# richox/orz

Measured on AMD Instinct MI355X. Metric: orz -l1 encode throughput (enwik8-shaped text, 100 MB, one 16 MiB block in flight), higher is better.
Workload: dtype u8

## Files before the change

### orz_amd/csrc/backend_hip.h

```cpp
#pragma once
#include <hip/hip_runtime.h>

#include <cxxabi.h>

#include <chrono>
#include <condition_variable>
#include <algorithm>
#include <atomic>
#include <cstring>
#include <map>
#include <mutex>
#include <rocprim/rocprim.hpp>
#include <stdexcept>
#include <string>
#include <type_traits>
#include <vector>

#include "orz_kernels.h"
#include "orz_parse.h"
#include "orz_symrank.h"

namespace orz {

#define ORZ_HIP_CHECK(expr)                                                                              \
// ... 32 lines not shown
        const uint32_t lo = (uint32_t)__builtin_amdgcn_readlane((int)(uint32_t)v, (int)src);
        const uint32_t hi = (uint32_t)__builtin_amdgcn_readlane((int)(uint32_t)(v >> 32), (int)src);
        return (uint64_t)lo | ((uint64_t)hi << 32);
    }
    __device__ __forceinline__ unsigned long long clock() const { return __builtin_amdgcn_s_memtime(); }
    __device__ __forceinline__ unsigned long long wallclock() const { return __builtin_amdgcn_s_memrealtime(); }
};
template <class K>
__global__ __launch_bounds__(64) void orz_wave_kernel(K k) {
    extern __shared__ __attribute__((aligned(16))) uint8_t orz_dyn_lds[];
    DevWave w{orz_dyn_lds};
    k(w);
}

template <class K>
__global__ __launch_bounds__(1024) void orz_group_kernel(K k, bool use_lds) {
    extern __shared__ __attribute__((aligned(16))) uint8_t orz_dyn_lds[];
    for (uint32_t ph = 0; ph < K::kPhases; ph++) {
        if (ph) {
            __threadfence_block();
            __syncthreads();
        }
        k.phase(ph, threadIdx.x, blockDim.x, orz_dyn_lds, use_lds);
    }
}

__global__ __launch_bounds__(256) void orz_rank_kernel(RankArgs a, uint32_t nchunks, uint32_t nvblk) {
    __shared__ uint32_t rows[(kRankChunk + 1) * 256];
    auto sync = [] __device__() { __syncthreads(); };
    if (blockIdx.x < nchunks) rank_chunk(a, blockIdx.x, threadIdx.x, rows, sync);
    else if (blockIdx.x < nchunks + nvblk)
        rebuild_summaries(a.vbits, a.v1, a.v2, a.nvwords, blockIdx.x - nchunks, threadIdx.x, (uint64_t*)rows, sync);
    else
        rebuild_summaries(a.kbits, a.k1, a.k2, a.nkwords, blockIdx.x - nchunks - nvblk, threadIdx.x, (uint64_t*)rows, sync);
}


struct FastEval;

class ParseTokens {
   public:
    static ParseTokens& of(int device) {
        static ParseTokens t[64];
        return t[device & 63];
    }
    void acquire() {
// ... 281 lines not shown
        static std::atomic<int> done[64];
        std::atomic<int>* d = device_ >= 0 && device_ < 64 ? &done[device_] : nullptr;
        if (d) {
            const int v = d->load(std::memory_order_acquire);
            if (v) return (hipError_t)(v - 1);
        }
        int cur = -1;
        ORZ_HIP_CHECK(hipGetDevice(&cur));
        if (cur != device_) ORZ_HIP_CHECK(hipSetDevice(device_));
        const hipError_t e = hipFuncSetAttribute(reinterpret_cast<const void*>(Kernel), hipFuncAttributeMaxDynamicSharedMemorySize, bytes);
        if (cur != device_) ORZ_HIP_CHECK(hipSetDevice(cur));
        if (d) d->store(1 + (int)e, std::memory_order_release);
        return e;
    }
    template <class K>
    void launch_waves(size_t nblocks, const K& k, size_t lds_bytes) {
        if (!nblocks) return;
        Bracket br(*this, profile_ ? KernelNames::of<K>() : 0);
        if (lds_bytes > 64 * 1024) {
            const hipError_t big = big_lds<&orz_wave_kernel<K>>(160 * 1024 - 256);
            if (big != hipSuccess) throw std::runtime_error(std::string("hipFuncSetAttribute(MaxDynamicSharedMemorySize): ") + hipGetErrorString(big));
        }
        hipLaunchKernelGGL(orz_wave_kernel<K>, dim3((unsigned)nblocks), dim3(64), lds_bytes, stream_, k);
        ORZ_HIP_CHECK(hipGetLastError());
    }
    template <class K>
    void launch_group(const K& k) {
        Bracket br(*this, profile_ ? KernelNames::of<K>() : 0);
        size_t lds = k.lds_bytes();
        const bool big_ok = big_lds<&orz_group_kernel<K>>((int)K::kLdsMax) == hipSuccess;
        if (lds > 64 * 1024 && !big_ok) lds = 0;
        hipLaunchKernelGGL(orz_group_kernel<K>, dim3(1), dim3(1024), lds, stream_, k, lds != 0);
        ORZ_HIP_CHECK(hipGetLastError());
    }
    void huffbuild(const HuffBuild& f) {
        if (f.nchunks) launch_waves((size_t)f.nchunks * 3, HuffWave{f}, HuffWave::lds_bytes());
    }
    void rank(const RankArgs& a, uint32_t nchunks) {
        const uint32_t nvblk = (a.nvwords + 4095) / 4096, nkblk = (a.nkwords + 4095) / 4096;
        hipLaunchKernelGGL(orz_rank_kernel, dim3(nchunks + nvblk + nkblk), dim3(256), 0, stream_, a, nchunks, nvblk);
        ORZ_HIP_CHECK(hipGetLastError());
    }
    void sort_pairs_u32(const uint32_t* kin, uint32_t* kout, const uint32_t* vin, uint32_t* vout, size_t n, int bits) {
        if (n == 0) return;
        Bracket br(*this, profile_ ? KernelNames::lib("(radix sort, pairs)") : 0);
        size_t sz = tmp_bytes_;
// ... 229 lines not shown
```

### orz_amd/csrc/orz_fast.h

```cpp
#pragma once
#include "orz_kernels.h"
#include "orz_parse.h"

namespace orz {

#if !defined(__HIPCC__)
inline unsigned long long g_far_stats[4] = {0, 0, 0, 0};
#endif

constexpr uint32_t kSub = 4096;
constexpr uint32_t kSeg64 = 64;
constexpr uint32_t kNSub = kNewMax / kSub + 2;
constexpr uint32_t kEntries = 240;

constexpr uint32_t kFastK = 32;
constexpr uint32_t kHistSub = (kPre + 1) / kSub;
constexpr uint32_t kRingMargin = 4;
constexpr uint32_t kFastTile = 262144;
constexpr uint32_t kFastRounds = 4;
constexpr uint32_t kSettledTile = 393216;
constexpr uint32_t kSettledTileDeep = 262144;
constexpr uint32_t kSettledRounds = 3;

struct FastArgs {
    const uint8_t* win;
    uint32_t len, n;
    uint32_t K, depth, lazy1, lazy2, tile;
    uint32_t dmax;
    uint32_t nent, nk;
    const uint32_t *idx, *epos, *kidx, *kpos, *krun;
    const uint8_t* rows;
    const uint8_t* rlen;
    const uint64_t* rdist;
    const uint64_t* wmask;
    const uint16_t* kmeta;
    const uint16_t* kw;
    const uint8_t* wsnap;
    const uint32_t* ORD;
    const uint64_t* stext;
    const uint32_t* runstart;
    const uint32_t* hpre;
    uint32_t far;
    uint32_t near;
    uint32_t near1;
    uint32_t extra;
    uint64_t* cl;
    uint32_t *ccnt, *cnew;
    uint32_t rounds;
    uint32_t* farv;
    uint64_t *vbits, *kbits;
    uint64_t* v1;
    uint64_t* k1;
    uint64_t* tbits;
    uint32_t* ev;
    uint8_t *ty, *nl, *pt;
    uint64_t* sbits;
    uint8_t *mfb, *efb;
    uint8_t* dirty;
// ... 166 lines not shown
            }
        }
        if (p < kPre) return;
        const uint32_t d = j - rs;
        rlen[p - kPre] = (uint8_t)(d < 255 ? d : 255);
    }
};
struct FastKw {
    const uint8_t* win;
    const uint32_t* kpos;
    uint32_t nk;
    uint16_t* kw;
    ORZ_HD void operator()(size_t s) const {
        if (s >= nk) return;
        const uint32_t u = kpos[s];
        kw[s] = (uint16_t)(win[u] | (win[u + 1] << 8));
    }
};
struct FastWordMasks {
    const uint32_t *kpos, *kkeys, *krun;
    const uint16_t* kw;
    const uint8_t* wsnap;
    uint32_t nk;
    uint64_t* wmask;
    uint16_t* kmeta;
    static size_t lds_bytes() { return 128 * 2; }
    template <class W>
    ORZ_D void operator()(W& w) const {
        uint16_t* kwL = (uint16_t*)w.lds();
        const uint32_t lane = w.lane();
        const int64_t base = (int64_t)w.block() * 64 - 64;
        for (uint32_t e = lane; e < 128; e += 64) {
            const int64_t s = base + e;
            kwL[e] = s >= 0 && s < (int64_t)nk ? kw[s] : 0;
        }
        w.sync();
        const uint32_t s = w.block() * 64 + lane;
        if (s >= nk) return;
        const uint32_t u = kpos[s];
        if (u < kPre) return;
        const uint32_t key = kkeys[s], rk = fast_min(64u, s - krun[key]);
        const uint32_t me = 64 + lane, wv = kwL[me];
        uint64_t m = 0;
        for (uint32_t t = 0; t < rk; t++) m |= (uint64_t)(kwL[me - 1 - t] == wv) << (63 - t);
        const uint32_t excl = rk && kpos[s - 1] == u - 1;
        const uint32_t snap = ((uint32_t)wsnap[key * 2] | ((uint32_t)wsnap[key * 2 + 1] << 8)) == wv;
        wmask[u - kPre] = m;
        kmeta[u - kPre] = (uint16_t)(rk | (excl << 7) | (snap << 8));
    }
};
struct HistCountWave {
    const uint8_t* win;
    const uint8_t* S;
    uint32_t* hcm;
    static size_t lds_bytes() { return 256 * 4; }
    template <class W>
    ORZ_D void operator()(W& w) const {
        uint32_t* cnt = (uint32_t*)w.lds();
        const uint32_t u = w.block(), lane = w.lane();
        for (uint32_t c = lane; c < 256; c += 64) cnt[c] = 0;
        w.sync();
        const uint32_t x0 = u * kSub + lane * 64;
        for (uint32_t k = 0; k < 64; k++) {
            const uint32_t x = x0 + k - 1;
            if (x0 + k == 0 || x < 1 || x >= kPre) continue;
            if (S[x]) atom_add32(&cnt[hash1(win, x - 1)], 1);
        }
        w.sync();
        for (uint32_t c = lane; c < 256; c += 64) hcm[(size_t)u * 256 + c] = cnt[c];
    }
};
// ... 40 lines not shown
        uint32_t v = gsum[(size_t)g * 256 + c];
        for (uint32_t r = g * 64; r < rows && r < g * 64 + 64; r++) {
            out[(size_t)r * 256 + c] = v;
            v += in[(size_t)r * 256 + c];
        }
        if (g * 64 + 64 >= rows) out[(size_t)rows * 256 + c] = v;
    }
};
constexpr uint32_t kRecText = 12;
ORZ_D uint32_t rec_pos(uint64_t hi) { return (uint32_t)(hi >> 32); }
ORZ_D uint32_t rec_lcp(uint64_t lo_a, uint64_t hi_a, uint64_t lo_b, uint64_t hi_b) {
    const uint64_t x0 = lo_a ^ lo_b;
    if (x0) return (uint32_t)ctz64(x0) >> 3;
    const uint32_t x1 = (uint32_t)(hi_a ^ hi_b);
    return x1 ? 8 + ((uint32_t)ctz64((uint64_t)x1) >> 3) : kRecText;
}
struct FastRowsWave {
    const uint8_t* win;
    const uint32_t* epos;
    const uint64_t* stext;
    const uint8_t* rlen;
    uint32_t nent, K;
    uint8_t* rows;
    uint64_t* rdist;
    static constexpr uint32_t kOutStride = 72;
    static size_t lds_bytes(uint32_t K) { return (size_t)(64 + K) * 16 + 64 * kOutStride; }
    template <class W>
    ORZ_D void operator()(W& w) const {
        uint64_t* t0 = (uint64_t*)w.lds();
        uint64_t* t1 = t0 + (64 + K);
        uint8_t* outL = (uint8_t*)(t1 + (64 + K));
        const uint32_t lane = w.lane();
        const int64_t base = (int64_t)w.block() * 64 - K;
        for (uint32_t e = lane; e < 64 + K; e += 64) {
            const int64_t s = base + e;
            uint64_t a = 0, b = 0;
            if (s >= 0 && s < (int64_t)nent) { a = stext[2 * s]; b = stext[2 * s + 1]; }
            t0[e] = a; t1[e] = b;
        }
        w.sync();
        const uint32_t me = K + lane;
        const uint32_t p = rec_pos(t1[me]);
        const bool mine = (int64_t)w.block() * 64 + lane < (int64_t)nent && p >= kPre;
        const uint32_t r = mine ? fast_min(K, rlen[p - kPre]) : 0;
        const uint64_t a0 = t0[me], a1 = t1[me];
        const uint64_t a2 = mine ? ldu64(win + p + kRecText) : 0;
        if (mine) {
            uint64_t codes = 0;
            for (uint32_t m = 0; m < 8; m++) {
                const uint32_t k = r ? fast_min(dist_sample(m), r - 1) : 0;
                const uint32_t code = r ? dist_code_up(p - rec_pos(t1[me - 1 - k])) : 255u;
                codes |= (uint64_t)code << (8 * m);
            }
            rdist[p - kPre] = codes;
        }
        const uint32_t cols = K < 64 ? K : 64;
        const uint32_t parts = cols / 16;
        for (uint32_t c0 = 0; c0 < K; c0 += cols) {
            for (uint32_t k0 = 0; k0 < cols; k0 += 8) {
                uint32_t ll[8], lq[8];
                uint64_t yy[8];
#pragma unroll
                for (uint32_t kk = 0; kk < 8; kk++) {
                    const uint32_t k = c0 + k0 + kk;
                    ll[kk] = 0; lq[kk] = 0;
                    if (k < r) {
                        const uint32_t e = me - 1 - k;
                        const uint64_t hi = t1[e];
                        ll[kk] = rec_lcp(t0[e], hi, a0, a1);
                        lq[kk] = rec_pos(hi);
                    }
                }
#pragma unroll
                for (uint32_t kk = 0; kk < 8; kk++) yy[kk] = ll[kk] == kRecText ? ldu64(win + lq[kk] + kRecText) : 0;
                uint64_t pack = 0;
#pragma unroll
                for (uint32_t kk = 0; kk < 8; kk++) {
// ... 251 lines not shown
                    else if (rnd == a.rounds) {
                        g_scan_hist[1][sb]++;
                        if (a.farv[i] != fv) { g_scan_hist[2][sb]++; g_scan_hist[3][popc64(wbits) < 63 ? popc64(wbits) : 63]++; }
                    }
                }
#endif
        }
        return fv;
    }
    ORZ_D uint32_t position_of(size_t tid) const {
        const uint32_t span = hi - lo, T = a.tile;
        if ((a.dbg & 2048) || span <= T) return lo + (uint32_t)tid;
        const uint32_t nch = (span + T - 1) / T, s_last = span - (nch - 1) * T;
        if (tid < s_last) return lo + (nch - 1) * T + (uint32_t)tid;
        const uint32_t u = (uint32_t)tid - s_last, k = u / T, off = u - k * T;
        const uint32_t c = k == 0 ? nch - 2 : k - 1;
        return lo + c * T + off;
    }
    ORZ_HD void operator()(size_t tid) const {
        const uint32_t p = position_of(tid);
        if (p >= hi) return;
        const uint8_t* win = a.win;
        const uint32_t i = p - kPre;
        const uint32_t rl = a.rlen[i];
        const bool first = p >= r1lo;
        const bool longrun = rl > kFastK;
        const uint32_t t = i / a.tile, rnd = step > t ? step - t : 0;
        bool scan = longrun && (rnd <= 1 || rnd == a.rounds);
        if (a.dbg & (12 | 128 | 256)) {
            if ((a.dbg & 8) || ((a.dbg & 4) && rnd > 1)) scan = false;
            if ((a.dbg & 128) && rnd <= 1) scan = false;
            if (a.dbg & 256) scan = longrun && (rnd == 2 || rnd == a.rounds);
        }
        if ((a.dbg & 16) && scan && rnd > 1) {
            const uint64_t sw = bits_at(a.sbits, (int64_t)i - 2);
            const bool rel = ((sw >> 2) & 1) || (((sw >> 1) & 1) && i >= 1 && a.ty[i - 1] == kTyMatch) || ((sw & 1) && i >= 2 && a.ty[i - 2] == kTyMatch);
            if (!rel) scan = false;
        }
        const bool dirty = a.dirty[i] != 0 || (a.dbg & 1);
        const uint32_t c = hash1(win, p - 1);
        const uint32_t* hz = a.hz + ((size_t)(i / kSub) * 256 + c) * 4;
        const uint32_t h4 = hz[0], h4was = hz[2];
        const bool need = p >= r2lo || dirty || scan;
#if !defined(__HIPCC__) && !defined(ORZ_EMU_THREADS)
        g_eval_stats[0]++;
        if (first) g_eval_stats[2]++; else if (dirty) g_eval_stats[3]++; else if (scan) g_eval_stats[4]++;
#endif
        if (!need && h4was == h4) return;
        const uint64_t codes = a.rdist[i];
        const DistBracket d4 = dist_valid(codes, p > h4 ? p - h4 : 0);
        bool moved = false;
        if (!first && h4was != h4) {
            const DistBracket o4 = dist_valid(codes, p > h4was ? p - h4was : 0);
            moved = o4.sure != d4.sure || o4.limit != d4.limit || d4.sure < fast_min(fast_min(kFastK, rl), d4.limit);
        }
        if (!need && !moved) return;
#if !defined(__HIPCC__) && !defined(ORZ_EMU_THREADS)
        g_eval_stats[1]++;
#endif
        const uint32_t j = a.idx[p], kj = a.kidx[p], r = fast_min(kFastK, rl);
        const uint32_t km = a.kmeta[i], rk = km & 0x7f;
        const uint64_t wm = a.wmask[i];
        const uint32_t h5 = hz[1];
        uint32_t rw[kFastK / 4];
        {
            const uint32_t* src = reinterpret_cast<const uint32_t*>(a.rows + (size_t)i * kFastK);
#pragma unroll
            for (uint32_t q = 0; q < kFastK / 16; q++) {
                if (r > q * 16) {
#pragma unroll
                    for (uint32_t d = 0; d < 4; d++) rw[q * 4 + d] = src[q * 4 + d];
                } else {
#pragma unroll
                    for (uint32_t d = 0; d < 4; d++) rw[q * 4 + d] = 0;
                }
            }
        }
        uint64_t mask = r ? bits_at(a.vbits, (int64_t)j - 64) : 0;
        uint64_t kmask = rk ? bits_at(a.kbits, (int64_t)kj - 64) : 0;
        if (r < 64) mask = r ? mask & (~0ull << (64 - r)) : 0;
        const uint64_t wbits = mask;
        const DistBracket d5 = dist_valid(codes, p > h5 ? p - h5 : 0);
        uint32_t v4 = count_from(d4, r, j, h4);
        if (a.dbg & 2) v4 = 64;
        const uint32_t span = fast_min(r, v4);
// ... 201 lines not shown
    uint32_t c0, nc;
    ORZ_HD void operator()(size_t tid) const {
        const uint32_t c = c0 + (uint32_t)(tid / kEntries), e = (uint32_t)(tid % kEntries);
        if (c >= c0 + nc) return;
        const uint32_t end = chunk_end(c, a.len);
        uint32_t x = kPre + c * kSub + e;
        while (x < end) {
            const uint32_t s = (x - kPre) / kSeg64;
            x = seg_end(s, a.len) + a.x0[x - kPre];
        }
        a.x1[(size_t)c * kEntries + e] = (uint8_t)(x >= end ? x - end : 0);
    }
};
ORZ_D uint32_t pad68(uint32_t x) { return (x >> 6) * 68 + (x & 63); }
ORZ_D void st8_pad68(uint8_t* tab, uint32_t x, uint64_t v) {
    uint32_t* d = reinterpret_cast<uint32_t*>(tab + pad68(x));
    d[0] = (uint32_t)v; d[1] = (uint32_t)(v >> 32);
}
struct PathUpWave {
    FastArgs a;
    uint32_t c0;
    uint32_t decide = 0, nup = 0;
    FastRetireDone done{};
    static size_t lds_bytes() { return 2 * 64 * 68 + 64; }
    template <class W>
    ORZ_D void operator()(W& w) const {
        if (decide && w.block() >= nup) {
            const uint32_t t = (w.block() - nup) * 64 + w.lane();
            done((size_t)t);
            return;
        }
        uint8_t* nlL = w.lds();
        uint8_t* x0L = nlL + 64 * 68 + 32;
        const uint32_t c = c0 + w.block() / 4, part = w.block() & 3, lane = w.lane();
        const uint32_t cs = kPre + c * kSub, clen = chunk_end(c, a.len) - cs;
        uint64_t w5[8][5];
        if (decide) {
#pragma unroll
            for (uint32_t k = 0; k < 8; k++) {
                const uint32_t x = (k * 64 + lane) * 8;
                const uint64_t* ew = reinterpret_cast<const uint64_t*>(a.ev + (cs - kPre) + (x < clen ? x : 0));
#pragma unroll
                for (uint32_t q = 0; q < 5; q++) w5[k][q] = ew[q];
            }
        }
#pragma unroll
        for (uint32_t k = 0; k < 8; k++) {
            const uint32_t x = (k * 64 + lane) * 8;
            if (!decide) {
                st8_pad68(nlL, x, x < clen ? *reinterpret_cast<const uint64_t*>(a.nl + (cs - kPre) + x) : 0);
                continue;
            }
            uint64_t nlw = 0, tyw = 0;
            if (x < clen) {
                const uint32_t i0 = (cs - kPre) + x;
                uint32_t e[10];
#pragma unroll
                for (uint32_t q = 0; q < 10; q++) {
                    const uint32_t v = (uint32_t)(w5[k][q >> 1] >> (32 * (q & 1)));
                    e[q] = cs + x + q < a.len ? v : 0;
                }
#pragma unroll
                for (uint32_t q = 0; q < 8; q++) {
                    const uint32_t p = cs + x + q;
                    const uint32_t d = p < a.len ? fast_decide(p, a.len, e[q], e[q + 1], e[q + 2]) : 0;
                    tyw |= (uint64_t)(d & 0xff) << (8 * q);
                    nlw |= (uint64_t)((d >> 8) & 0xff) << (8 * q);
                }
                if ((x >> 10) == part) {
                    if (x + 8 <= clen) {
                        *reinterpret_cast<uint64_t*>(a.ty + i0) = tyw;
                        *reinterpret_cast<uint64_t*>(a.nl + i0) = nlw;
                    } else {
                        for (uint32_t q = 0; x + q < clen; q++) { a.ty[i0 + q] = (uint8_t)(tyw >> (8 * q)); a.nl[i0 + q] = (uint8_t)(nlw >> (8 * q)); }
                    }
                }
            }
            st8_pad68(nlL, x, nlw);
        }
        w.sync();
        {
            const uint32_t s0 = lane * 64;
            if (s0 < clen) {
                const uint32_t s1 = fast_min(s0 + 64, clen), sl = s1 - s0;
                uint32_t adv[16];
                const uint32_t* row = reinterpret_cast<const uint32_t*>(nlL + lane * 68);
#pragma unroll
                for (uint32_t q = 0; q < 16; q++) adv[q] = row[q];
                uint8_t* xrow = x0L + lane * 68;
#pragma unroll
                for (uint32_t k = 0; k < 64; k++) {
                    const uint32_t p = 63 - k;
                    if (p < sl) {
                        const uint32_t d = (adv[p >> 2] >> (8 * (p & 3))) & 0xff, x = p + (d ? d : 1);
                        xrow[p] = x >= sl ? (uint8_t)(x - sl) : xrow[x];
                    }
                }
            }
        }
        w.sync();
        for (uint32_t k = part * 2; k < part * 2 + 2; k++) {
            const uint32_t x = (k * 64 + lane) * 8;
            if (x >= clen) continue;
            const uint32_t* src = reinterpret_cast<const uint32_t*>(x0L + pad68(x));
            *reinterpret_cast<uint64_t*>(a.x0 + (cs - kPre) + x) = (uint64_t)src[0] | ((uint64_t)src[1] << 32);
        }
        w.sync();
        if (lane < 60) {
            const uint32_t e = part * 60 + lane;
            uint32_t x = e;
            while (x < clen) {
                const uint32_t s1 = fast_min(((x >> 6) + 1) * 64, clen);
                x = s1 + x0L[pad68(x)];
            }
            a.x1[(size_t)c * kEntries + e] = (uint8_t)(x - clen);
        }
    }
};
struct PathMarkWave {
    FastArgs a;
    uint32_t c0;
    static constexpr uint32_t kTab = 64 * 68 + 32;
    static size_t lds_bytes() { return 3 * kTab + (65 * 68 + 12) + 256 * 4; }
    template <class W>
    ORZ_D void operator()(W& w) const {
        uint8_t* nlL = w.lds();
        uint8_t* x0L = nlL + kTab;
        uint8_t* tyL = x0L + kTab;
        uint8_t* wL = tyL + kTab;
        uint32_t* cnt = (uint32_t*)(wL + 65 * 68 + 12);
        const uint32_t c = c0 + w.block(), lane = w.lane();
        const uint32_t cs = kPre + c * kSub, clen = chunk_end(c, a.len) - cs;
        for (uint32_t k = lane; k < 256; k += 64) cnt[k] = 0;
        {
            uint64_t v[8], u[8], t[8], b[8];
#pragma unroll
            for (uint32_t k = 0; k < 8; k++) {
                const uint32_t x = (k * 64 + lane) * 8;
// ... 966 lines not shown
```

### orz_amd/csrc/orz_stream.h

```cpp
#pragma once
#include <algorithm>
#include <atomic>
#include <cstdio>
#include <cstdlib>
#include <cstring>
#include <stdexcept>
#include <string>
#include <vector>

#include "orz_fast.h"
#include "orz_kernels.h"
#include "orz_parse.h"
#include "orz_verify.h"

namespace orz {

struct ItemTrace {
    std::vector<uint32_t> block, pos, src;
    std::vector<uint16_t> sym, ctx, rank, rob;
    std::vector<uint8_t> unl, enc, al, mlen;
    void clear() { block.clear(); pos.clear(); src.clear(); sym.clear(); ctx.clear(); rank.clear(); rob.clear(); unl.clear(); enc.clear(); al.clear(); mlen.clear(); }
};

struct FastTableCapture {
// ... 316 lines not shown
        n_ = m;
    }
    void push_back(uint8_t b) {
        if (n_ == cap_) reserve(cap_ ? cap_ * 2 : 4096);
        p_[n_++] = b;
    }
    size_t size() const { return n_; }
    bool empty() const { return n_ == 0; }
    uint8_t* data() { return p_; }
    const uint8_t* data() const { return p_; }
    void clear() { n_ = 0; }
    uint8_t* release() {
        if (!p_) reserve(1);
        uint8_t* q = p_;
        p_ = nullptr;
        n_ = cap_ = 0;
        return q;
    }

   private:
    uint8_t* p_ = nullptr;
    size_t n_ = 0, cap_ = 0;
};

template <class BE>
class StreamEncoder {
   public:
    static constexpr size_t kChunkCapWords = (size_t)kChunkItems * 40 / 32 + 8192;
    static constexpr uint32_t kMaxChunks = 17;
    static constexpr uint32_t kNumKeys = 256 * kHash;
    static constexpr uint32_t kDirtyWords = kNumKeys / 64 + 1;
    static constexpr int kFirstPasses = 12;
    static constexpr uint32_t kRepairGrid = 16384;

    StreamEncoder(BE& be, Cfg cfg, uint32_t seg_size = 62, uint32_t win_segs = 3072, bool fast = false,
                  uint32_t fast_tile = kFastTile, uint32_t fast_rounds = kFastRounds)
        : be_(be), cfg_(cfg), seg_(seg_size), wsegs_(win_segs), fast_(fast), ftile_(fast_tile), frounds_(fast_rounds) {
        if (fast_) {
            if (ftile_ < kSub || ftile_ % kSub || ftile_ > kNewMax) throw std::runtime_error("fast tile must be a multiple of 4096 in [4096, 16777216]");
            if (frounds_ < 1 || frounds_ > 64) throw std::runtime_error("fast rounds must be in [1, 64]");
            fK_ = kFastK;
            sched_auto_ = ftile_ == kFastTile && frounds_ == kFastRounds;
            if (cfg.depth > 20) sched_tile_ = kSettledTileDeep;
            if (const char* sc = getenv("ORZ_FAST_SCHED")) {
                unsigned t = 0, r = 0;
                if (sscanf(sc, "%ux%u", &t, &r) == 2 && t >= kSub && t % kSub == 0 && t <= kNewMax && r >= 1 && r <= 64) { sched_tile_ = t; sched_rounds_ = r; }
// ... 55 lines not shown
            kbits_ = take<uint64_t>(kNewMax / 64 + 2);
            k1_ = take<uint64_t>(kNewMax / 4096 + 2);
            k2_ = take<uint64_t>(kNewMax / 262144 + 2);
            if (!fast_) {
                srec_ = take<SlotRec>(kWLen);
                exitst_ = take<uint64_t>((size_t)nseg_max_ + 2);
                hist_ = take<uint8_t>((size_t)ring_ * 256);
                base_ = take<uint32_t>((size_t)ring_ * 256);
                ctl_ = take<ParseCtl>(1);
                partial_ = take<uint32_t>((size_t)2 * (wsegs_ / kRankChunk + 1) * 256);
            } else {
                const size_t nn = (size_t)kNewMax + 512;
                frows_ = take<uint8_t>((size_t)kNewMax * fK_ + 64, false);
                frlen_ = take<uint8_t>(nn);
                fstext_ = take<uint64_t>((size_t)kWLen * 2, false);
                fkw_ = take<uint16_t>(nn);
                fev_ = take<uint32_t>(nn, false);
                fty_ = take<uint8_t>(nn);
                fnl_ = take<uint8_t>(nn);
                fpt_ = take<uint8_t>(nn);
                fmf_ = take<uint8_t>(nn);
                fef_ = take<uint8_t>(nn);
                fdirty_ = take<uint8_t>(nn);
                frdist_ = take<uint64_t>(nn, false);
                fwmask_ = take<uint64_t>(nn, false);
                fkmeta_ = take<uint16_t>(nn);
                fhz_ = take<uint32_t>((size_t)(kNSub + 2) * 256 * 4);
                fhcm_ = take<uint32_t>((size_t)kHistSub * 256);
                fhpre_ = take<uint32_t>((size_t)(kHistSub + 1) * 256);
                fgsum_ = take<uint32_t>((size_t)(kNSub / 64 + 4) * 256);
                fdiag_ = take<unsigned long long>(64);
                fx0_ = take<uint8_t>(nn);
                fx1_ = take<uint8_t>((size_t)(kNSub + 2) * kEntries);
                fx2_ = take<uint8_t>((size_t)(kNewMax / kSub + 4) * kEntries);
                fsbits_ = take<uint64_t>(kNewMax / 64 + 16);
                fcentry_ = take<uint32_t>(kNSub + 2);
                ftentry_ = take<uint32_t>(kNewMax / kSub + 4);
                fcm_ = take<uint32_t>((size_t)(kNSub + 2) * 256);
                fcp_ = take<uint32_t>((size_t)(kNSub + 2) * 256);
                fcut_ = take<uint32_t>(nn);
                frdirty_ = take<uint64_t>((size_t)2 * kDirtyWords);
                flaste_ = take<uint32_t>(nn);
                fctl_ = take<FastCtl>(1);
                fcok_ = take<uint32_t>(512);
                ffarv_ = take<uint32_t>(nn, false);
                fcl_ = take<uint64_t>((size_t)kWLen * 2, false);
                fccnt_ = take<uint32_t>(kNumKeys + 1);
                fcnew_ = take<uint32_t>(kNumKeys + 1);
            }
// ... 321 lines not shown
    void capture_tables(uint32_t n, uint32_t nent, const uint32_t* slot_keys, const uint32_t* word_keys) {
        FastTableCapture& c = *tables;
        const uint32_t nhist = nent - n, nk = n + 1;
        c.tab.clear();
        be_.sync();
        auto put = [&](const char* name, const void* dev, size_t bytes) {
            c.tab.emplace_back(name, std::vector<uint8_t>(bytes));
            be_.d2h(c.tab.back().second.data(), dev, bytes);
        };
        const uint64_t sc[8] = {n, nhist, nent, nk, fK_, stats.in_bytes, stats.blocks, kPre};
        c.tab.emplace_back("scalars", std::vector<uint8_t>((const uint8_t*)sc, (const uint8_t*)sc + sizeof sc));
        put("hpos", hpos_, (size_t)nhist * 4);
        put("wsnap", wsnap_, 65536);
        put("epos", epos_, (size_t)nent * 4);
        put("keys", slot_keys, (size_t)nent * 4);
        put("idx", idx_ + kPre, (size_t)n * 4);
        put("runstart", runstart_, (size_t)kNumKeys * 4);
        put("rlen", frlen_, n);
        put("vbits", vbits_, ((size_t)nent / 64 + 2) * 8);
        put("stext", fstext_, (size_t)nent * 16);
        put("cl", fcl_, (size_t)nent * 16);
        put("ccnt", fccnt_, (size_t)kNumKeys * 4);
        put("rows", frows_, (size_t)n * fK_);
        put("rdist", frdist_, (size_t)n * 8);
        put("kpos", kpos_, (size_t)nk * 4);
        put("kkeys", word_keys, (size_t)nk * 4);
        put("krun", krun_, 32768 * 4);
        put("kw", fkw_, (size_t)nk * 2);
        put("wmask", fwmask_, (size_t)n * 8);
        put("kmeta", fkmeta_, (size_t)n * 2);
        put("hcm", fhcm_, (size_t)kHistSub * 256 * 4);
        put("hpre", fhpre_, (size_t)(kHistSub + 1) * 256 * 4);
        c.taken = true;
        c.arm = -1;
    }

    template <class OutT>
    void fast_parse(uint32_t n, uint32_t len, uint32_t nent, const uint32_t* slot_keys, const uint32_t* word_keys, OutT& out) {
        const uint8_t* win = dwin();
        const uint32_t nk = n + 1, K = fK_, nsub = (n + kSub - 1) / kSub, nvw = nent / 64 + 2;
        be_.launch(nk, FastKw{win, kpos_, nk, fkw_});
        be_.launch_waves(((size_t)nk + 63) / 64, FastWordMasks{kpos_, word_keys, krun_, fkw_, wsnap_, nk, fwmask_, fkmeta_}, FastWordMasks::lds_bytes());
        if (!stream_start_) be_.launch_waves(kHistSub, HistCountWave{win, S_, fhcm_}, HistCountWave::lds_bytes());
        col_scan(fhcm_, kHistSub, fhpre_);
        uint64_t* stext = fstext_;
        {
            FastSlotInitWave si{epos_, slot_keys, runstart_, nent, vbits_, frlen_};
            si.win = win; si.stext = stext; si.cl = fcl_; si.ccnt = fccnt_;
            be_.launch_waves(((size_t)nent + 63) / 64, si, 0);
        }
        be_.timed_begin(2);
        be_.launch_waves(((size_t)nent + 63) / 64, FastRowsWave{win, epos_, stext, frlen_, nent, K, frows_, frdist_}, FastRowsWave::lds_bytes(K));
        be_.timed_end(2);
        if (tables && tables->arm >= 0 && (uint64_t)tables->arm == stats.blocks) capture_tables(n, nent, slot_keys, word_keys);
        FastArgs a;
        a.win = win; a.len = len; a.n = n; a.K = K; a.depth = (uint32_t)cfg_.depth; a.lazy1 = (uint32_t)cfg_.lazy1;
        a.lazy2 = (uint32_t)cfg_.lazy2; a.tile = ftile_; a.dmax = dmax_; a.nent = nent; a.nk = nk;
        a.idx = idx_; a.epos = epos_; a.kidx = kidx_; a.kpos = kpos_; a.krun = krun_; a.rows = frows_; a.rlen = frlen_;
        a.rdist = frdist_; a.wmask = fwmask_; a.kmeta = fkmeta_; a.hpre = fhpre_;
        a.kw = fkw_; a.wsnap = wsnap_; a.ORD = ORD_; a.stext = fstext_; a.runstart = runstart_; a.farv = ffarv_;
        a.far = getenv("ORZ_FAST_FAR") ? (uint32_t)atoi(getenv("ORZ_FAST_FAR")) : 16384; a.vbits = vbits_; a.kbits = kbits_; a.v1 = v1_; a.ev = fev_;
        a.ty = fty_; a.nl = fnl_; a.pt = fpt_; a.sbits = fsbits_; a.mfb = fmf_; a.efb = fef_; a.dirty = fdirty_; a.hz = fhz_;
        a.x0 = fx0_; a.x1 = fx1_; a.x2 = fx2_;
        a.cl = fcl_; a.ccnt = fccnt_; a.cnew = fcnew_; a.rounds = frounds_;
        static const bool repair_lists = !(getenv("ORZ_FAST_REPAIR") && !strcmp(getenv("ORZ_FAST_REPAIR"), "grid"));
        const uint32_t nsub_max = kNewMax / kSub + 2;
        uint8_t* scratch = reinterpret_cast<uint8_t*>(entA_);
        auto carve = [&](size_t bytes) { uint8_t* q = scratch; scratch += (bytes + 255) & ~(size_t)255; return q; };
        uint16_t* mlist = reinterpret_cast<uint16_t*>(carve((size_t)nsub_max * kSubMatches * 2));
        uint16_t* wlist = reinterpret_cast<uint16_t*>(carve((size_t)nsub_max * kSubWords * 2));
        uint32_t* mcnt = reinterpret_cast<uint32_t*>(carve((size_t)nsub_max * 4));
        uint32_t* wcnt = reinterpret_cast<uint32_t*>(carve((size_t)nsub_max * 4));
        uint32_t* cutlist = reinterpret_cast<uint32_t*>(carve(((size_t)kNewMax / kMinLen + 64) * 4));
        uint32_t* fixlist = reinterpret_cast<uint32_t*>(carve(((size_t)kNewMax / 2 + 64) * 4));
        uint32_t* wextra = reinterpret_cast<uint32_t*>(carve(((size_t)kNewMax / 2 + 64) * 4));
        const size_t tbits_bytes = ((size_t)kNewMax / 64 + 8) * 8, kdirty_bytes = 512 * 8;
        uint64_t* tbits = reinterpret_cast<uint64_t*>(carve(tbits_bytes));
        uint64_t* kdirty = reinterpret_cast<uint64_t*>(carve(kdirty_bytes));
        if ((size_t)(scratch - reinterpret_cast<uint8_t*>(entA_)) > (size_t)kWLen * 8) throw std::runtime_error("repair lists do not fit the sort buffer");
        a.k1 = k1_; a.tbits = tbits;

        a.near = getenv("ORZ_FAST_NEAR") ? (uint32_t)atoi(getenv("ORZ_FAST_NEAR")) : 16;
// ... 58 lines not shown
                bool on;
                ~CaptureGuard() { if (on) be.graph_capture_abort(); }
            } capture{be_, use_graph && !replayed};
            if (capture.on) be_.graph_capture_begin();
            if (replayed) stats.sweeps += ntile + R - 1;
            for (uint32_t step = 1; step <= ntile + R - 1 && !replayed; step++) {
                const uint32_t t_lo = step > R ? step - R : 0, t_hi = std::min(step - 1, ntile - 1);
                const uint32_t lo = kPre + t_lo * T;
                const uint32_t hi = (uint32_t)std::min<uint64_t>(len, (uint64_t)kPre + (uint64_t)(t_hi + 1) * T);
                const uint32_t hi2 = std::min(len, hi + 2);
                be_.timed_begin();
                const uint32_t r1lo = step <= ntile ? kPre + t_hi * T : hi;
                const uint32_t r2lo = step >= 2 && step - 2 < ntile ? kPre + (step - 2) * T : (step < 2 ? kPre : hi);
                const uint32_t mark_hi = step - 1 < ntile ? kPre + (step - 1) * T : len;
                const uint32_t cline = kPre + (step > R ? step - R : 0) * T;
                be_.launch(hi2 - lo, FastEval{a, lo, hi2, r1lo, r2lo, step, cline});
                be_.timed_end();
                const uint32_t c0 = t_lo * cpt, nc = (hi - (kPre + c0 * kSub) + kSub - 1) / kSub, nt = t_hi - t_lo + 1;
                be_.timed_begin(3);
                if (fused_steps) {
                    const bool had_retire = step - 1 >= R && step - 1 < ntile + R - 1;
                    const uint32_t plo = had_retire ? kPre + (step - 1 - R) * T : kPre, phi = had_retire ? (uint32_t)std::min<uint64_t>(len, (uint64_t)plo + T) : kPre;
                    PathUpWave up{a, c0};
                    up.decide = 1; up.nup = nc * 4; up.done = FastRetireDone{a, plo, phi, fcut_};
                    be_.launch_waves((size_t)nc * 4 + (phi - plo + 63) / 64, up, PathUpWave::lds_bytes());
                } else {
                    be_.launch(hi - lo, FastDecide{a, lo, hi});
                    be_.launch_waves((size_t)nc * 4, PathUpWave{a, c0}, PathUpWave::lds_bytes());
                }
                be_.timed_end(3);
                be_.launch_group(PathTileDown{a, t_lo, nt});
                be_.launch_waves(nc, PathMarkWave{a, c0}, PathMarkWave::lds_bytes());
                const uint32_t fhi = std::min(len, hi + 240);
                const FastFlip ff{a, lo, fhi, t_hi + 1, mark_hi, step >= R ? (uint32_t)std::min<uint64_t>(len, (uint64_t)lo + T) : 0, &fctl_->lastflips};
                const uint32_t ext = std::min(cpt + 1, nsub - std::min(nsub, c0 + nc));
                const FastPrefix fp{a, c0, c0 + nc, ext, cpt, step >= R ? std::min(c0 + cpt, c0 + nc) : c0};
                const FastHorizon fh{a, c0, c0 + nc + ext - 1};
                const bool retire = step >= R && step < ntile + R - 1;
                const uint32_t rlo = retire ? kPre + (step - R) * T : kPre, rhi = retire ? (uint32_t)std::min<uint64_t>(len, (uint64_t)rlo + T) : kPre;
                if (fused_steps) {
                    const uint32_t nflip = fhi - lo + 1, nret = rhi - rlo;
                    be_.launch_waves(flip_blocks(nflip) + 256, FlipPrefixWave{ff, fp, nflip}, FlipPrefixWave::lds_bytes());
                    be_.launch_waves((size_t)(nret + 63) / 64 + (fh.threads() + 63) / 64, RetireHorizonWave{FastRetire{a, rlo, rhi, fcut_}, fh, nret}, 0);
                } else {
                    be_.launch((size_t)fhi - lo + 1, ff);
                    be_.launch_waves(256, fp, 0);
                    be_.launch(fh.threads(), fh);
                    if (retire) {
                        be_.launch(rhi - rlo, FastRetire{a, rlo, rhi, fcut_});
                        be_.launch(rhi - rlo, FastRetireDone{a, rlo, rhi, fcut_});
                    }
// ... 495 lines not shown
    }
    void release_all() {
        for (void* p : owned_) if (p) be_.free(p);
        owned_.clear();
        be_.release_arena();
    }
    void release_token() {
        if (token_held_) { token_held_ = false; be_.parse_token_release(); }
    }
    bool token_held_ = false;
    bool pre_items_valid_ = false;
    uint32_t pre_two_[2] = {0, 0};
    std::vector<void*> owned_;
    BE& be_;
    Cfg cfg_;
    uint32_t seg_, wsegs_, ring_ = 0, nseg_max_ = 0, dmax_ = 0;
    bool fast_ = false;
    uint32_t ftile_ = kFastTile, frounds_ = kFastRounds, fK_ = kFastK;
    bool sched_auto_ = false, settled_next_ = false;
    uint32_t sched_tile_ = kSettledTile, sched_rounds_ = kSettledRounds;
    bool lead_block_ = false;
    uint8_t *frows_ = nullptr, *frlen_ = nullptr, *fty_ = nullptr, *fnl_ = nullptr, *fpt_ = nullptr, *fmf_ = nullptr, *fef_ = nullptr,
            *fx0_ = nullptr, *fx1_ = nullptr, *fx2_ = nullptr, *fdirty_ = nullptr;
    uint16_t *fkw_ = nullptr, *fkmeta_ = nullptr;
    uint64_t *frdist_ = nullptr, *fwmask_ = nullptr;
    uint32_t *fhz_ = nullptr, *fhcm_ = nullptr, *fhpre_ = nullptr, *fgsum_ = nullptr;
    unsigned long long* fdiag_ = nullptr;
    uint32_t *fev_ = nullptr, *fcentry_ = nullptr, *ftentry_ = nullptr, *fcm_ = nullptr, *fcp_ = nullptr, *fcut_ = nullptr,
             *flaste_ = nullptr, *fcok_ = nullptr, *ffarv_ = nullptr;
    uint64_t *fsbits_ = nullptr, *fstext_ = nullptr, *frdirty_ = nullptr, *fcl_ = nullptr;
    uint32_t *fccnt_ = nullptr, *fcnew_ = nullptr;
    FastCtl* fctl_ = nullptr;
    FastCtl hfin_{};
    uint8_t lt_carry_ = kTyLit;
    bool stream_start_ = true;
    struct TailSet {
        uint32_t* ipos = nullptr;
        uint16_t *isym = nullptr, *ictx = nullptr, *irank = nullptr, *irob = nullptr, *grank = nullptr, *skey = nullptr;
        uint8_t *iunl = nullptr, *ienc = nullptr, *ial = nullptr;
        uint32_t *gsym = nullptr, *sperm = nullptr, *blen = nullptr, *bscan = nullptr, *rstart = nullptr;
        uint32_t* hw = nullptr;
        uint8_t* hl = nullptr;
        uint16_t* hc = nullptr;
        uint32_t *hdrbits = nullptr, *tot = nullptr, *out = nullptr, *srflags = nullptr;
        bool pending = false;
        bool framed = false;
        uint32_t cap = 0;
        uint32_t nitems = 0, nchunks = 0, len = 0, block = 0;
// ... 129 lines not shown
```

Baseline: 492.5.

## Pack per-position match records into 32-byte structs and run PathUp as 256-thread blocks

Replaces the separate rdist, wmask, kmeta arrays and the idx/kidx/rlen lookups in the eval kernel with one 32-byte record per position (run half and word half). The eval step can then fetch everything with two 16-byte loads instead of several scattered ones. PathUpWave is also moved from four independent 64-lane blocks per chunk into one 256-thread block that runs three barrier-separated phases. Each wave now only decides its own quarter, instead of every wave recomputing the decisions for the whole chunk. Costs: more memory per position (32 bytes versus 18), an extra per-record write of slot indices, and block-wide barriers in PathUp.

```diff
diff --git a/orz_amd/csrc/backend_hip.h b/orz_amd/csrc/backend_hip.h
--- a/orz_amd/csrc/backend_hip.h
+++ b/orz_amd/csrc/backend_hip.h
@@ -78,6 +78,25 @@
             __syncthreads();
         }
         k.phase(ph, threadIdx.x, blockDim.x, orz_dyn_lds, use_lds);
+    }
+}
+
+struct DevQuad {
+    uint8_t* lds_;
+    __device__ __forceinline__ uint32_t lane() const { return threadIdx.x & 63; }
+    __device__ __forceinline__ uint32_t wave() const { return threadIdx.x >> 6; }
+    __device__ __forceinline__ uint32_t block() const { return blockIdx.x; }
+    __device__ __forceinline__ uint8_t* lds() const { return lds_; }
+    __device__ __forceinline__ void sync() const { __syncthreads(); }
+};
+template <class K>
+__global__ __launch_bounds__(256) void orz_quad_kernel(K k) {
+    extern __shared__ __attribute__((aligned(16))) uint8_t orz_dyn_lds[];
+    DevQuad w{orz_dyn_lds};
+#pragma unroll
+    for (uint32_t ph = 0; ph < K::kPhases; ph++) {
+        if (ph) __syncthreads();
+        k.phase(ph, w);
     }
 }
 
@@ -405,6 +424,13 @@
             if (big != hipSuccess) throw std::runtime_error(std::string("hipFuncSetAttribute(MaxDynamicSharedMemorySize): ") + hipGetErrorString(big));
         }
         hipLaunchKernelGGL(orz_wave_kernel<K>, dim3((unsigned)nblocks), dim3(64), lds_bytes, stream_, k);
+        ORZ_HIP_CHECK(hipGetLastError());
+    }
+    template <class K>
+    void launch_quads(size_t nblocks, const K& k, size_t lds_bytes) {
+        if (!nblocks) return;
+        Bracket br(*this, profile_ ? KernelNames::of<K>() : 0);
+        hipLaunchKernelGGL(orz_quad_kernel<K>, dim3((unsigned)nblocks), dim3(256), lds_bytes, stream_, k);
         ORZ_HIP_CHECK(hipGetLastError());
     }
     template <class K>
diff --git a/orz_amd/csrc/orz_fast.h b/orz_amd/csrc/orz_fast.h
--- a/orz_amd/csrc/orz_fast.h
+++ b/orz_amd/csrc/orz_fast.h
@@ -21,6 +21,14 @@
 constexpr uint32_t kSettledTile = 393216;
 constexpr uint32_t kSettledTileDeep = 262144;
 constexpr uint32_t kSettledRounds = 3;
+
+struct alignas(16) FastRecHalf {
+    uint64_t m;
+    uint32_t slot;
+    uint32_t meta;
+};
+struct FastRec { FastRecHalf run, word; };
+static_assert(sizeof(FastRec) == 32, "two 16-byte loads");
 
 struct FastArgs {
     const uint8_t* win;
@@ -31,9 +39,7 @@
     const uint32_t *idx, *epos, *kidx, *kpos, *krun;
     const uint8_t* rows;
     const uint8_t* rlen;
-    const uint64_t* rdist;
-    const uint64_t* wmask;
-    const uint16_t* kmeta;
+    const FastRec* rec;
     const uint16_t* kw;
     const uint8_t* wsnap;
     const uint32_t* ORD;
@@ -246,8 +252,7 @@
     const uint16_t* kw;
     const uint8_t* wsnap;
     uint32_t nk;
-    uint64_t* wmask;
-    uint16_t* kmeta;
+    FastRec* rec;
     static size_t lds_bytes() { return 128 * 2; }
     template <class W>
     ORZ_D void operator()(W& w) const {
@@ -269,8 +274,7 @@
         for (uint32_t t = 0; t < rk; t++) m |= (uint64_t)(kwL[me - 1 - t] == wv) << (63 - t);
         const uint32_t excl = rk && kpos[s - 1] == u - 1;
         const uint32_t snap = ((uint32_t)wsnap[key * 2] | ((uint32_t)wsnap[key * 2 + 1] << 8)) == wv;
-        wmask[u - kPre] = m;
-        kmeta[u - kPre] = (uint16_t)(rk | (excl << 7) | (snap << 8));
+        rec[u - kPre].word = FastRecHalf{m, s, rk | (excl << 7) | (snap << 8)};
     }
 };
 struct HistCountWave {
@@ -357,7 +361,7 @@
     const uint8_t* rlen;
     uint32_t nent, K;
     uint8_t* rows;
-    uint64_t* rdist;
+    FastRec* rec;
     static constexpr uint32_t kOutStride = 72;
     static size_t lds_bytes(uint32_t K) { return (size_t)(64 + K) * 16 + 64 * kOutStride; }
     template <class W>
@@ -377,7 +381,7 @@
         const uint32_t me = K + lane;
         const uint32_t p = rec_pos(t1[me]);
         const bool mine = (int64_t)w.block() * 64 + lane < (int64_t)nent && p >= kPre;
-        const uint32_t r = mine ? fast_min(K, rlen[p - kPre]) : 0;
+        const uint32_t rl = mine ? rlen[p - kPre] : 0, r = fast_min(K, rl);
         const uint64_t a0 = t0[me], a1 = t1[me];
         const uint64_t a2 = mine ? ldu64(win + p + kRecText) : 0;
         if (mine) {
@@ -387,7 +391,7 @@
                 const uint32_t code = r ? dist_code_up(p - rec_pos(t1[me - 1 - k])) : 255u;
                 codes |= (uint64_t)code << (8 * m);
             }
-            rdist[p - kPre] = codes;
+            rec[p - kPre].run = FastRecHalf{codes, w.block() * 64 + lane, rl};
         }
         const uint32_t cols = K < 64 ? K : 64;
         const uint32_t parts = cols / 16;
@@ -685,7 +689,8 @@
         if (p >= hi) return;
         const uint8_t* win = a.win;
         const uint32_t i = p - kPre;
-        const uint32_t rl = a.rlen[i];
+        const FastRecHalf run = a.rec[i].run, word = a.rec[i].word;
+        const uint32_t rl = run.meta;
         const bool first = p >= r1lo;
         const bool longrun = rl > kFastK;
         const uint32_t t = i / a.tile, rnd = step > t ? step - t : 0;
@@ -710,7 +715,7 @@
         if (first) g_eval_stats[2]++; else if (dirty) g_eval_stats[3]++; else if (scan) g_eval_stats[4]++;
 #endif
         if (!need && h4was == h4) return;
-        const uint64_t codes = a.rdist[i];
+        const uint64_t codes = run.m;
         const DistBracket d4 = dist_valid(codes, p > h4 ? p - h4 : 0);
         bool moved = false;
         if (!first && h4was != h4) {
@@ -721,9 +726,9 @@
 #if !defined(__HIPCC__) && !defined(ORZ_EMU_THREADS)
         g_eval_stats[1]++;
 #endif
-        const uint32_t j = a.idx[p], kj = a.kidx[p], r = fast_min(kFastK, rl);
-        const uint32_t km = a.kmeta[i], rk = km & 0x7f;
-        const uint64_t wm = a.wmask[i];
+        const uint32_t j = run.slot, kj = word.slot, r = fast_min(kFastK, rl);
+        const uint32_t km = word.meta, rk = km & 0x7f;
+        const uint64_t wm = word.m;
         const uint32_t h5 = hz[1];
         uint32_t rw[kFastK / 4];
         {
@@ -971,52 +976,52 @@
     uint32_t c0;
     uint32_t decide = 0, nup = 0;
     FastRetireDone done{};
+    static constexpr uint32_t kPhases = 3;
     static size_t lds_bytes() { return 2 * 64 * 68 + 64; }
     template <class W>
-    ORZ_D void operator()(W& w) const {
+    ORZ_D void phase(uint32_t ph, W& w) const {
         if (decide && w.block() >= nup) {
-            const uint32_t t = (w.block() - nup) * 64 + w.lane();
-            done((size_t)t);
+            if (ph == 0) done((size_t)(w.block() - nup) * 256 + w.wave() * 64 + w.lane());
             return;
         }
         uint8_t* nlL = w.lds();
         uint8_t* x0L = nlL + 64 * 68 + 32;
-        const uint32_t c = c0 + w.block() / 4, part = w.block() & 3, lane = w.lane();
+        const uint32_t c = c0 + w.block(), part = w.wave(), lane = w.lane();
         const uint32_t cs = kPre + c * kSub, clen = chunk_end(c, a.len) - cs;
-        uint64_t w5[8][5];
-        if (decide) {
-#pragma unroll
-            for (uint32_t k = 0; k < 8; k++) {
-                const uint32_t x = (k * 64 + lane) * 8;
-                const uint64_t* ew = reinterpret_cast<const uint64_t*>(a.ev + (cs - kPre) + (x < clen ? x : 0));
-#pragma unroll
-                for (uint32_t q = 0; q < 5; q++) w5[k][q] = ew[q];
-            }
-        }
-#pragma unroll
-        for (uint32_t k = 0; k < 8; k++) {
-            const uint32_t x = (k * 64 + lane) * 8;
-            if (!decide) {
-                st8_pad68(nlL, x, x < clen ? *reinterpret_cast<const uint64_t*>(a.nl + (cs - kPre) + x) : 0);
-                continue;
-            }
-            uint64_t nlw = 0, tyw = 0;
-            if (x < clen) {
-                const uint32_t i0 = (cs - kPre) + x;
-                uint32_t e[10];
-#pragma unroll
-                for (uint32_t q = 0; q < 10; q++) {
-                    const uint32_t v = (uint32_t)(w5[k][q >> 1] >> (32 * (q & 1)));
-                    e[q] = cs + x + q < a.len ? v : 0;
+        if (ph == 0) {
+            uint64_t w5[2][5];
+            if (decide) {
+#pragma unroll
+                for (uint32_t k = 0; k < 2; k++) {
+                    const uint32_t x = ((part * 2 + k) * 64 + lane) * 8;
+                    const uint64_t* ew = reinterpret_cast<const uint64_t*>(a.ev + (cs - kPre) + (x < clen ? x : 0));
+#pragma unroll
+                    for (uint32_t q = 0; q < 5; q++) w5[k][q] = ew[q];
                 }
-#pragma unroll
-                for (uint32_t q = 0; q < 8; q++) {
-                    const uint32_t p = cs + x + q;
-                    const uint32_t d = p < a.len ? fast_decide(p, a.len, e[q], e[q + 1], e[q + 2]) : 0;
-                    tyw |= (uint64_t)(d & 0xff) << (8 * q);
-                    nlw |= (uint64_t)((d >> 8) & 0xff) << (8 * q);
+            }
+#pragma unroll
+            for (uint32_t k = 0; k < 2; k++) {
+                const uint32_t x = ((part * 2 + k) * 64 + lane) * 8;
+                if (!decide) {
+                    st8_pad68(nlL, x, x < clen ? *reinterpret_cast<const uint64_t*>(a.nl + (cs - kPre) + x) : 0);
+                    continue;
                 }
-                if ((x >> 10) == part) {
+                uint64_t nlw = 0, tyw = 0;
+                if (x < clen) {
+                    const uint32_t i0 = (cs - kPre) + x;
+                    uint32_t e[10];
+#pragma unroll
+                    for (uint32_t q = 0; q < 10; q++) {
+                        const uint32_t v = (uint32_t)(w5[k][q >> 1] >> (32 * (q & 1)));
+                        e[q] = cs + x + q < a.len ? v : 0;
+                    }
+#pragma unroll
+                    for (uint32_t q = 0; q < 8; q++) {
+                        const uint32_t p = cs + x + q;
+                        const uint32_t d = p < a.len ? fast_decide(p, a.len, e[q], e[q + 1], e[q + 2]) : 0;
+                        tyw |= (uint64_t)(d & 0xff) << (8 * q);
+                        nlw |= (uint64_t)((d >> 8) & 0xff) << (8 * q);
+                    }
                     if (x + 8 <= clen) {
                         *reinterpret_cast<uint64_t*>(a.ty + i0) = tyw;
                         *reinterpret_cast<uint64_t*>(a.nl + i0) = nlw;
@@ -1024,13 +1029,11 @@
                         for (uint32_t q = 0; x + q < clen; q++) { a.ty[i0 + q] = (uint8_t)(tyw >> (8 * q)); a.nl[i0 + q] = (uint8_t)(nlw >> (8 * q)); }
                     }
                 }
-            }
-            st8_pad68(nlL, x, nlw);
-        }
-        w.sync();
-        {
+                st8_pad68(nlL, x, nlw);
+            }
+        } else if (ph == 1) {
             const uint32_t s0 = lane * 64;
-            if (s0 < clen) {
+            if (part == 0 && s0 < clen) {
                 const uint32_t s1 = fast_min(s0 + 64, clen), sl = s1 - s0;
                 uint32_t adv[16];
                 const uint32_t* row = reinterpret_cast<const uint32_t*>(nlL + lane * 68);
@@ -1046,23 +1049,22 @@
                     }
                 }
             }
-        }
-        w.sync();
-        for (uint32_t k = part * 2; k < part * 2 + 2; k++) {
-            const uint32_t x = (k * 64 + lane) * 8;
-            if (x >= clen) continue;
-            const uint32_t* src = reinterpret_cast<const uint32_t*>(x0L + pad68(x));
-            *reinterpret_cast<uint64_t*>(a.x0 + (cs - kPre) + x) = (uint64_t)src[0] | ((uint64_t)src[1] << 32);
-        }
-        w.sync();
-        if (lane < 60) {
-            const uint32_t e = part * 60 + lane;
-            uint32_t x = e;
-            while (x < clen) {
-                const uint32_t s1 = fast_min(((x >> 6) + 1) * 64, clen);
-                x = s1 + x0L[pad68(x)];
-            }
-            a.x1[(size_t)c * kEntries + e] = (uint8_t)(x - clen);
+        } else {
+            for (uint32_t k = part * 2; k < part * 2 + 2; k++) {
+                const uint32_t x = (k * 64 + lane) * 8;
+                if (x >= clen) continue;
+                const uint32_t* src = reinterpret_cast<const uint32_t*>(x0L + pad68(x));
+                *reinterpret_cast<uint64_t*>(a.x0 + (cs - kPre) + x) = (uint64_t)src[0] | ((uint64_t)src[1] << 32);
+            }
+            if (lane < 60) {
+                const uint32_t e = part * 60 + lane;
+                uint32_t x = e;
+                while (x < clen) {
+                    const uint32_t s1 = fast_min(((x >> 6) + 1) * 64, clen);
+                    x = s1 + x0L[pad68(x)];
+                }
+                a.x1[(size_t)c * kEntries + e] = (uint8_t)(x - clen);
+            }
         }
     }
 };
diff --git a/orz_amd/csrc/orz_stream.h b/orz_amd/csrc/orz_stream.h
--- a/orz_amd/csrc/orz_stream.h
+++ b/orz_amd/csrc/orz_stream.h
@@ -362,6 +362,34 @@
     uint8_t* p_ = nullptr;
     size_t n_ = 0, cap_ = 0;
 };
+
+template <class W> struct QuadOnWaveCtx {
+    W& w;
+    uint32_t blk, wv;
+    uint32_t lane() const { return w.lane(); }
+    uint32_t wave() const { return wv; }
+    uint32_t block() const { return blk; }
+    uint8_t* lds() const { return w.lds(); }
+    void sync() { w.sync(); }
+};
+template <class K> struct QuadOnWave {
+    const K* k;
+    uint32_t blk, wv, ph;
+    template <class W> void operator()(W& w) const {
+        QuadOnWaveCtx<W> q{w, blk, wv};
+        k->phase(ph, q);
+    }
+};
+template <class BE, class K>
+auto launch_quads_on(BE& be, size_t nblocks, const K& k, size_t lds_bytes, int) -> decltype(be.launch_quads(nblocks, k, lds_bytes)) {
+    be.launch_quads(nblocks, k, lds_bytes);
+}
+template <class BE, class K>
+void launch_quads_on(BE& be, size_t nblocks, const K& k, size_t lds_bytes, long) {
+    for (size_t b = nblocks; b-- > 0;)
+        for (uint32_t ph = 0; ph < K::kPhases; ph++)
+            for (uint32_t wv = 0; wv < 4; wv++) be.launch_waves(1, QuadOnWave<K>{&k, (uint32_t)b, wv, ph}, lds_bytes);
+}
 
 template <class BE>
 class StreamEncoder {
@@ -463,9 +491,7 @@
                 fmf_ = take<uint8_t>(nn);
                 fef_ = take<uint8_t>(nn);
                 fdirty_ = take<uint8_t>(nn);
-                frdist_ = take<uint64_t>(nn, false);
-                fwmask_ = take<uint64_t>(nn, false);
-                fkmeta_ = take<uint16_t>(nn);
+                frec_ = reinterpret_cast<FastRec*>((reinterpret_cast<uintptr_t>(take<FastRec>(nn + 1, false)) + 31) & ~(uintptr_t)31);
                 fhz_ = take<uint32_t>((size_t)(kNSub + 2) * 256 * 4);
                 fhcm_ = take<uint32_t>((size_t)kHistSub * 256);
                 fhpre_ = take<uint32_t>((size_t)(kHistSub + 1) * 256);
@@ -833,13 +859,20 @@
         put("cl", fcl_, (size_t)nent * 16);
         put("ccnt", fccnt_, (size_t)kNumKeys * 4);
         put("rows", frows_, (size_t)n * fK_);
-        put("rdist", frdist_, (size_t)n * 8);
+        std::vector<FastRec> recs(n);
+        be_.d2h(recs.data(), frec_, (size_t)n * sizeof(FastRec));
+        auto field = [&](const char* name, size_t width, auto get) {
+            c.tab.emplace_back(name, std::vector<uint8_t>((size_t)n * width));
+            uint8_t* dst = c.tab.back().second.data();
+            for (uint32_t i = 0; i < n; i++) { const uint64_t v = get(recs[i]); std::memcpy(dst + (size_t)i * width, &v, width); }
+        };
+        field("rdist", 8, [](const FastRec& r) { return r.run.m; });
         put("kpos", kpos_, (size_t)nk * 4);
         put("kkeys", word_keys, (size_t)nk * 4);
         put("krun", krun_, 32768 * 4);
         put("kw", fkw_, (size_t)nk * 2);
-        put("wmask", fwmask_, (size_t)n * 8);
-        put("kmeta", fkmeta_, (size_t)n * 2);
+        field("wmask", 8, [](const FastRec& r) { return r.word.m; });
+        field("kmeta", 2, [](const FastRec& r) { return (uint64_t)r.word.meta; });
         put("hcm", fhcm_, (size_t)kHistSub * 256 * 4);
         put("hpre", fhpre_, (size_t)(kHistSub + 1) * 256 * 4);
         c.taken = true;
@@ -851,7 +884,7 @@
         const uint8_t* win = dwin();
         const uint32_t nk = n + 1, K = fK_, nsub = (n + kSub - 1) / kSub, nvw = nent / 64 + 2;
         be_.launch(nk, FastKw{win, kpos_, nk, fkw_});
-        be_.launch_waves(((size_t)nk + 63) / 64, FastWordMasks{kpos_, word_keys, krun_, fkw_, wsnap_, nk, fwmask_, fkmeta_}, FastWordMasks::lds_bytes());
+        be_.launch_waves(((size_t)nk + 63) / 64, FastWordMasks{kpos_, word_keys, krun_, fkw_, wsnap_, nk, frec_}, FastWordMasks::lds_bytes());
         if (!stream_start_) be_.launch_waves(kHistSub, HistCountWave{win, S_, fhcm_}, HistCountWave::lds_bytes());
         col_scan(fhcm_, kHistSub, fhpre_);
         uint64_t* stext = fstext_;
@@ -861,14 +894,14 @@
             be_.launch_waves(((size_t)nent + 63) / 64, si, 0);
         }
         be_.timed_begin(2);
-        be_.launch_waves(((size_t)nent + 63) / 64, FastRowsWave{win, epos_, stext, frlen_, nent, K, frows_, frdist_}, FastRowsWave::lds_bytes(K));
+        be_.launch_waves(((size_t)nent + 63) / 64, FastRowsWave{win, epos_, stext, frlen_, nent, K, frows_, frec_}, FastRowsWave::lds_bytes(K));
         be_.timed_end(2);
         if (tables && tables->arm >= 0 && (uint64_t)tables->arm == stats.blocks) capture_tables(n, nent, slot_keys, word_keys);
         FastArgs a;
         a.win = win; a.len = len; a.n = n; a.K = K; a.depth = (uint32_t)cfg_.depth; a.lazy1 = (uint32_t)cfg_.lazy1;
         a.lazy2 = (uint32_t)cfg_.lazy2; a.tile = ftile_; a.dmax = dmax_; a.nent = nent; a.nk = nk;
         a.idx = idx_; a.epos = epos_; a.kidx = kidx_; a.kpos = kpos_; a.krun = krun_; a.rows = frows_; a.rlen = frlen_;
-        a.rdist = frdist_; a.wmask = fwmask_; a.kmeta = fkmeta_; a.hpre = fhpre_;
+        a.rec = frec_; a.hpre = fhpre_;
         a.kw = fkw_; a.wsnap = wsnap_; a.ORD = ORD_; a.stext = fstext_; a.runstart = runstart_; a.farv = ffarv_;
         a.far = getenv("ORZ_FAST_FAR") ? (uint32_t)atoi(getenv("ORZ_FAST_FAR")) : 16384; a.vbits = vbits_; a.kbits = kbits_; a.v1 = v1_; a.ev = fev_;
         a.ty = fty_; a.nl = fnl_; a.pt = fpt_; a.sbits = fsbits_; a.mfb = fmf_; a.efb = fef_; a.dirty = fdirty_; a.hz = fhz_;
@@ -973,11 +1006,11 @@
                     const bool had_retire = step - 1 >= R && step - 1 < ntile + R - 1;
                     const uint32_t plo = had_retire ? kPre + (step - 1 - R) * T : kPre, phi = had_retire ? (uint32_t)std::min<uint64_t>(len, (uint64_t)plo + T) : kPre;
                     PathUpWave up{a, c0};
-                    up.decide = 1; up.nup = nc * 4; up.done = FastRetireDone{a, plo, phi, fcut_};
-                    be_.launch_waves((size_t)nc * 4 + (phi - plo + 63) / 64, up, PathUpWave::lds_bytes());
+                    up.decide = 1; up.nup = nc; up.done = FastRetireDone{a, plo, phi, fcut_};
+                    launch_quads_on(be_, (size_t)nc + (phi - plo + 255) / 256, up, PathUpWave::lds_bytes(), 0);
                 } else {
                     be_.launch(hi - lo, FastDecide{a, lo, hi});
-                    be_.launch_waves((size_t)nc * 4, PathUpWave{a, c0}, PathUpWave::lds_bytes());
+                    launch_quads_on(be_, nc, PathUpWave{a, c0}, PathUpWave::lds_bytes(), 0);
                 }
                 be_.timed_end(3);
                 be_.launch_group(PathTileDown{a, t_lo, nt});
@@ -1519,8 +1552,8 @@
     bool lead_block_ = false;
     uint8_t *frows_ = nullptr, *frlen_ = nullptr, *fty_ = nullptr, *fnl_ = nullptr, *fpt_ = nullptr, *fmf_ = nullptr, *fef_ = nullptr,
             *fx0_ = nullptr, *fx1_ = nullptr, *fx2_ = nullptr, *fdirty_ = nullptr;
-    uint16_t *fkw_ = nullptr, *fkmeta_ = nullptr;
-    uint64_t *frdist_ = nullptr, *fwmask_ = nullptr;
+    uint16_t* fkw_ = nullptr;
+    FastRec* frec_ = nullptr;
     uint32_t *fhz_ = nullptr, *fhcm_ = nullptr, *fhpre_ = nullptr, *fgsum_ = nullptr;
     unsigned long long* fdiag_ = nullptr;
     uint32_t *fev_ = nullptr, *fcentry_ = nullptr, *ftentry_ = nullptr, *fcm_ = nullptr, *fcp_ = nullptr, *fcut_ = nullptr,
```

New measurement: 495.8, median of 2. About the same (+0.7%).
